# corelab-src/dacapo

Hardware: AMD Instinct MI355X
Metric: NTT/s (NTT-equivalents over one run() of the ResNet HEVM program, nt=2^14) (higher is better)
Workload: dtype u64; 1 GPU; ResNet-20 (SiLU) HEVM program traced from the reference's examples/benchmarks/ResNet.py with its resnet20.silu.model weights, nt=2^14 slots, N=2^15, 14 x 60-bit primes (SEAL_HEVM.cpp:39-53); one independent ciphertext stream per GPU; streams_per_gpu=1, parallelism=replicas x1 (no collective in the op path)

## Files before the change

dacapo_amd/csrc/fused_ks.hip:

```cpp
#include "ks_mac.hpp"

namespace dacapo {

struct SrcStrided {
    const u64 *base;
    long stride;
    int prime_base, period;
    __device__ int prime(int z) const { return prime_base + z % period; }
    __device__ u64 load(int z, int g, int) const { return base[(long)z * stride + g]; }
};
template <int E>
__device__ __forceinline__ void rs_operand(u64 (&v)[E], const int (&g)[E], const RsItem &it, const SumSrc *__restrict__ srcs, int p, int i,
                                           size_t N, const DModulus &M)
{
    if (it.count == 0) {
        const u64 *x = it.src.limb(p, i, N);
#pragma unroll
        for (int j = 0; j < E; j++) v[j] = x[g[j]];
    } else {
        u64 s[E];
        Acc128 a[E];
#pragma unroll
        for (int j = 0; j < E; j++) s[j] = 0, a[j].clear();
        int n_plain = 0, n_prod = 0;
// ... 624 lines not shown
    const int z = blockIdx.y, k = z % t, b = z / t;
    const size_t N = (size_t)1 << logN;
    const double ratio = items[b].ratio;
    const u64 *cf = pt + (size_t)b * ELL * N;
    u64 *out = ptx + (size_t)z * N;
    const DModulus M = mods[k];
    ntt_tile<K, LOGE, true, false, false>(
        M, tw + ((size_t)k << logN), logN, blockIdx.x,
        [=](int g) { return residue_of_double(reencoded_coeff_fixed<ELL>(cf, (size_t)g, N, mods, crt, ratio), M); },
        [=](int g, u64 v) { out[g] = v; }, lds);
}

template <int K, int LOGE>
__global__ __launch_bounds__(kTileThreads) void f_frows_boot_final_kernel(const u64 *__restrict__ ptx, const BootItem *__restrict__ items,
                                                                           int t, const DModulus *__restrict__ mods,
                                                                           const u64 *__restrict__ tw, int logN)
{
    __shared__ __attribute__((aligned(16))) u64 lds[TileGeo<LOGE>::LDS_ELEMS];
    const int z = blockIdx.y, i = z % t;
    const size_t N = (size_t)1 << logN;
    const BootItem it = items[z / t];
    const DModulus M = mods[i];
    const u64 *in = ptx + (size_t)z * N;
    const u64 *z0 = it.zenc + (size_t)i * N, *z1 = it.zenc + ((size_t)t + i) * N;
    u64 *o0 = it.dst.limb(0, i, N), *o1 = it.dst.limb(1, i, N);
    ntt_tile<K, LOGE, false, false, true>(
        M, tw + ((size_t)i << logN), logN, blockIdx.x, [=](int g) { return in[g]; },
        [=](int g, u64 v) {
            o0[g] = addmod(v, z0[g], M.q);
            o1[g] = z1[g];
        },
        lds);
}

template <class Src>
static void launch_irows(const Context &c, Src src, u64 *out, long out_stride, int count, hipStream_t s)
{
    DC_GEO_SWITCH(c.k2, count, DC_LAUNCH((f_irows_kernel<KK, LE, Src>), grid, dim3(kTileThreads), 0, s, src, out, out_stride,
                                                  c.d_mods, c.d_itw, c.logN));
// ... 49 lines not shown
{
    DC_GEO_SWITCH(c.k2, B * ell, DC_LAUNCH((f_irows_boot_kernel<KK, LE>), grid, dim3(kTileThreads), 0, s, items, srcs, sk, ell, out,
                                                    c.d_mods, c.d_itw, c.logN));
}
void f_boot_reencode_fcols(const Context &c, const u64 *pt, u64 *ptx, const BootItem *items, int B, int ell, int t, CrtDev crt,
                           hipStream_t s)
{
    if (ell == 1) {
        DC_GEO_SWITCH(c.k1, B * t, DC_LAUNCH((f_boot_reencode_fcols_kernel<KK, LE, 1>), grid, dim3(kTileThreads), 0, s, pt, ptx, items,
                                                      t, c.d_mods, crt, c.d_tw, c.logN));
    } else {
        fprintf(stderr, "[dacapo_amd] f_boot_reencode_fcols: source level %d not instantiated\n", ell);
        abort();
    }
}
void f_frows_boot_final(const Context &c, const u64 *ptx, const BootItem *items, int B, int t, hipStream_t s)
{
    DC_GEO_SWITCH(c.k2, B * t, DC_LAUNCH((f_frows_boot_final_kernel<KK, LE>), grid, dim3(kTileThreads), 0, s, ptx, items, t,
                                                  c.d_mods, c.d_tw, c.logN));
}

void f_ks_frows_mac(const Context &c, int mode, const u64 *ext, const u64 *target, const KsItem *items, const u64 *shared_key, u64 *acc,
                    int B, int ell, hipStream_t s, bool fold_base)
{
    const u64 *pmod = (fold_base && mode == 0) ? c.d_pmod : nullptr;
    const KsMacShape sh = ks_mac_shape(c, ell, B);
    ks_mac_dispatch(c.k2, sh, [&](auto k, auto le, auto merge) {
        constexpr int KK = decltype(k)::value, LE = decltype(le)::value;
        constexpr bool MG = decltype(merge)::value;
        if (mode == 0)
            DC_LAUNCH((f_ks_frows_mac_kernel<KK, LE, 0, MG>), sh.grid, dim3(kTileThreads), 0, s, ext, target, items, shared_key, acc, ell, c.K,
                      c.d_mods, c.d_tw, c.d_itw, c.logN, pmod, sh.items_fast);
        else
            DC_LAUNCH((f_ks_frows_mac_kernel<KK, LE, 1, MG>), sh.grid, dim3(kTileThreads), 0, s, ext, target, items, shared_key, acc, ell, c.K,
// ... 102 lines not shown
```

dacapo_amd/csrc/hevm_vm.hip:

```cpp
#include "hevm_vm.hpp"

#include "../../include/dacapo_ckks.h"
#include "c_api_types.hpp"
#include "chacha.hpp"
#include "seal_serial.hpp"

#include <math.h>
#include <string.h>
#include <sys/random.h>

#include <algorithm>
#include <cmath>
#include <chrono>
#include <fstream>
#include <iostream>

namespace dacapo {

constexpr int kVmThreads = 256;

constexpr int kRngCoefs = 8;

__device__ __forceinline__ int rng_cbd(u64 w)
{
// ... 39 lines not shown

__global__ __launch_bounds__(kVmThreads) void sample_small_kernel(u64 *__restrict__ out, size_t N, int limbs, int cbd, ChaChaKey key,
                                                                   u64 object, u32 domain, const DModulus *__restrict__ mods)
{
    const size_t blk = (size_t)blockIdx.x * kVmThreads + threadIdx.x;
    u64 w[kRngCoefs];
    rng_words8(key, object, blk, 0, 0, domain, w);
    int v[kRngCoefs];
#pragma unroll
    for (int e = 0; e < kRngCoefs; e++) v[e] = cbd ? rng_cbd(w[e]) : rng_ternary(w[e]);
    for (int i = 0; i < limbs; i++) store_small8(out + (size_t)i * N + blk * kRngCoefs, v, mods[i].q);
}

__global__ __launch_bounds__(kVmThreads) void sample_enc_batch_kernel(u64 *__restrict__ out, size_t N, int cnt, ChaChaKey key, u64 object0,
                                                                       const DModulus *__restrict__ mods,
                                                                       const u64 *__restrict__ epoch)
{
    const int b = blockIdx.y / 3, z = blockIdx.y % 3;
    const size_t blk = (size_t)blockIdx.x * kVmThreads + threadIdx.x;
    u64 w[kRngCoefs];
    rng_words8(key, object0 + (u64)b, blk, *epoch, 0, RNG_ENC_U + (u32)z, w);
    int v[kRngCoefs];
#pragma unroll
    for (int e = 0; e < kRngCoefs; e++) v[e] = z ? rng_cbd(w[e]) : rng_ternary(w[e]);
    for (int i = 0; i < cnt; i++) store_small8(out + (((size_t)b * 3 + z) * cnt + i) * N + blk * kRngCoefs, v, mods[i].q);
}

__global__ void chacha_blocks_kernel(u32 *__restrict__ out, ChaChaKey key, u64 counter, u64 nonce, int blocks)
{
    const int b = blockIdx.x * blockDim.x + threadIdx.x;
    if (b >= blocks) return;
    u32 o[16];
    chacha20_block(key, counter + (u64)b, nonce, o);
    for (int i = 0; i < 16; i++) out[b * 16 + i] = o[i];
}

// ... 317 lines not shown
    encoder.reset(new HostEncoder(logN));
    use_plan = option(OPT_PLAN) != 0;
    plan_graph = option(OPT_PLAN_GRAPH) != 0;
    plan_dag = option(OPT_PLAN_GRAPH) == 2;
    plan_lanes = option(OPT_PLAN_LANES) >= 2 ? 2 : 1;
    host_encoder = option(OPT_HOST_ENCODER) != 0;
    fold_rescale_into_boot = option(OPT_FOLD_RESCALE_BOOT) != 0;
    lazy_sums = option(OPT_HYB_LAZY_SUM) != 0;
    double_hoist = (lazy_sums && option(OPT_HYB_DOUBLE_HOIST) != 0) || ks_lazy == 2;
    max_batch = std::max(1, (int)option(OPT_MAX_BATCH));
    chain_fusion = option(OPT_CHAIN_FUSION) != 0;
    secret_weight = (int)option(OPT_SECRET_HW);
    boot_secret_weight = (int)option(OPT_BOOT_SECRET_HW);
    rot_compose = option(OPT_ROT_COMPOSE) != 0;
    online_encode = option(OPT_ONLINE_ENCODE) != 0 && use_plan && !host_encoder;
    lanes.resize(1);
    DC_HIP_CHECK(hipStreamCreateWithFlags(&lanes[0].stream, hipStreamNonBlocking));
    lanes[0].ws = ctx->ws0;
    lanes[0].boot_plain.d = dalloc((size_t)ctx->max_level() * ctx->N);
    lanes[0].boot_plain.level = ctx->max_level();
    DC_HIP_CHECK(vm_malloc(&d_epoch, 8));
    DC_HIP_CHECK(hipMemset(d_epoch, 0, 8));
    cur = 0;
}

void HEVM::gen_kswitch_key(u64 *key, const u64 *new_key, u64 key_id) { gen_kswitch_key_in(*ctx, key, keys.sk, new_key, key_id); }

void HEVM::gen_kswitch_key_in(Context &c, u64 *key, const u64 *key_sk, const u64 *new_key, u64 key_id)
{
    const size_t N = c.N;
    const int K = c.K;
    const dim3 gu((unsigned)(N / (kRngCoefs * kVmThreads)), (unsigned)K), gs((unsigned)(N / (kRngCoefs * kVmThreads))),
        g2((unsigned)(N / (2 * kVmThreads)), (unsigned)K);
    const int L = c.max_level();
    for (int j = 0; j < c.key_digits(); j++) {
        u64 *c0 = key + (size_t)j * 2 * K * N, *c1 = c0 + (size_t)K * N;
        const u64 object = key_id * 64 + (u64)j;
// ... 735 lines not shown
    const size_t N = c.N;
    const int ell = pt.level, cnt = ell + 1;
    if (!keys.pk) {
        fprintf(stderr, "[dacapo_amd] encrypt: this VM has no public key\n");
        abort();
    }
    if (test_zero_enc) {
        DC_HIP_CHECK(hipMemcpyAsync(dst.data, pt.d, (size_t)ell * N * 8, hipMemcpyDeviceToDevice, S()));
        DC_HIP_CHECK(hipMemsetAsync(dst.data + dst.poly_stride, 0, (size_t)ell * N * 8, S()));
        dst.level = ell, dst.scale = pt.scale;
        return;
    }
    u64 *ue = W().ks_ext;
    const CtView tmp{ dst.data, (long)dst.poly_stride };
    DC_LAUNCH(sample_enc_batch_kernel, dim3((unsigned)(N / (kRngCoefs * kVmThreads)), 3), dim3(kVmThreads), 0, S(), ue, N, cnt,
                       rng.secret, enc_counter++, c.d_mods, d_epoch);
    launch_ntt(c, false, ue, (long)N, 3 * cnt, nullptr, 0, cnt, S());
    DC_LAUNCH(pk_encrypt_kernel, dim3((unsigned)(N / (2 * kVmThreads)), (unsigned)cnt, 2), dim3(kVmThreads), 0, S(),
                       tmp.p, tmp.poly_stride, keys.pk, (long)c.K * (long)N, ue, ue + (size_t)cnt * N, (long)cnt * (long)N, N, c.d_mods);
    rescale_fused(c, W(), tmp, tmp, cnt, pt.d, S());
    dst.level = ell;
    dst.scale = pt.scale;
}

void HEVM::encrypt(int64_t i, const double *dat, int len)
{
    Plain pt;
    encode_internal(pt, dat, (size_t)len, (int)arg_level.at((size_t)i), (int)arg_scale.at((size_t)i));
    hevm_ctxt &r = reg((size_t)i);
    reg_base[(size_t)i] = home[(size_t)i];
    r.data = reg_base[(size_t)i] + (size_t)sel * (size_t)2 * ctx->K * ctx->N;
// ... 450 lines not shown
    const CrtTables &tb = crt_tables(ell);
    u64 *pt = W().ks_tmp;
    u64 *lohi = W().ks_digits;
    f_irows_decrypt(c, src, keys.sk, ell, pt, S());
    launch_ntt_cols_inv(c, pt, (long)N, ell, nullptr, 0, 0, S());
    const CrtDev cd{ tb.inv, tb.mmod, tb.hmod, tb.hdig, tb.mdbl };
    DC_LAUNCH(reencode_kernel, dim3((unsigned)((N / 2 + kVmThreads) / kVmThreads)), dim3(kVmThreads), 0, S(), lohi,
                       lohi + N, pt, ell, N, c.d_mods, cd, new_scale / src_scale);
    Plain ptx{ lanes[cur].boot_plain.d, target_level, new_scale };
    DC_LAUNCH(lift_i128_kernel, dim3((unsigned)(N / kVmThreads), (unsigned)target_level), dim3(kVmThreads), 0, S(),
                       ptx.d, lohi, lohi + N, N, c.d_mods);
    launch_ntt(c, false, ptx.d, (long)N, target_level, nullptr, 0, 0, S());
    encrypt_plain(dst, ptx);
}

void HEVM::plan_zero_encrypt(int first, int B, int t, hipStream_t s)
{
    Context &c = *ctx;
    const size_t N = c.N;
    const int cnt = t + 1;
    if (!keys.pk) {
        fprintf(stderr, "[dacapo_amd] bootstrap: this VM has no public key\n");
        abort();
    }
    Plan &P = plan;
    DC_LAUNCH(sample_enc_batch_kernel, dim3((unsigned)(N / (kRngCoefs * kVmThreads)), (unsigned)(3 * B)), dim3(kVmThreads), 0, s,
                       P.boot_ue, N, cnt, rng.secret, ((u64)1 << 32) + (u64)first, c.d_mods, d_epoch);
    launch_ntt(c, false, P.boot_ue, (long)N, 3 * cnt * B, nullptr, 0, cnt, s);
    DC_LAUNCH(pk_encrypt_batch_kernel, dim3((unsigned)(N / (2 * kVmThreads)), (unsigned)cnt, (unsigned)(2 * B)), dim3(kVmThreads),
                       0, s, P.boot_tmp, keys.pk, (long)c.K * (long)N, P.boot_ue, cnt, N, c.d_mods);
    b_rescale(c, P.ws[0], P.d_boot_rs + first, B, cnt, s);
}

void HEVM::plan_boot_step(int first, int B, int ell, int t, int lane, hipStream_t s, const Handoff &h)
{
    Context &c = *ctx;
    const size_t N = c.N;
    if (!keys.sk) {
        fprintf(stderr, "[dacapo_amd] bootstrap: needs a full VM (secret + public key)\n");
        abort();
    }
    Plan &P = plan;
    const BootItem *items = P.d_boot + first;
    const CrtTables &tb = crt_tables(ell);
    const CrtDev cd{ tb.inv, tb.mmod, tb.hmod, tb.hdig, tb.mdbl };
    u64 *pt = P.boot_pt[lane], *ptx = P.boot_ptx[lane];
    if (h.in)
        pt = const_cast<u64 *>(h.in);
    else
        f_irows_decrypt_items(c, items, P.d_sum_srcs, keys.sk, ell, pt, B, s);
    launch_ntt_cols_inv(c, pt, (long)N, B * ell, nullptr, 0, ell, s);
    if (ell == 1)
        f_boot_reencode_fcols(c, pt, ptx, items, B, ell, t, cd, s);
    else {
        DC_LAUNCH(reencode_lift_batch_kernel, dim3((unsigned)((N / 2 + kVmThreads) / kVmThreads), (unsigned)B), dim3(kVmThreads), 0,
                           s, ptx, pt, items, ell, t, N, c.d_mods, cd);
        launch_ntt_cols_fwd(c, ptx, (long)N, B * t, nullptr, 0, t, s);
    }
    f_frows_boot_final(c, ptx, items, B, t, s);
}

void HEVM::dispatch(const WireOp &op)
{
    switch (op.opcode) {
    case 1: op_rotate(op.dst, op.lhs, (int16_t)op.rhs); break;
    case 2: op_negate(op.dst, op.lhs); break;
    case 3: op_rescale(op.dst, op.lhs); break;
    case 4: op_modswitch(op.dst, op.lhs, (int16_t)op.rhs); break;
    case 5: fprintf(stderr, "This VM does not support native upscale op\n"); abort();
    case 6: op_addcc(op.dst, op.lhs, op.rhs); break;
    case 7: op_addcp(op.dst, op.lhs, op.rhs); break;
    case 8: op_mulcc(op.dst, op.lhs, op.rhs); break;
    case 9: op_mulcp(op.dst, op.lhs, op.rhs); break;
    case 10: op_bootstrap(op.dst, op.lhs, op.rhs); break;
// ... 12 lines not shown
    n_hops = n_decomp = 0;
    t_bootstrap = 0.0;
    int i = (int)((header.hevm_header_size + config.config_body_length) / 8), j = 0;
    for (const WireOp &op : ops) {
        if (debug) {
            std::cout << std::endl;
            std::cout << std::oct << i++ << " " << std::dec << j++ << std::endl;
            std::cout << "opcode [" << op.opcode << "], dst [" << op.dst << "], lhs [" << op.lhs << "], rhs [" << op.rhs << "]"
                      << std::endl;
        }
        if (op.opcode <= 10) op_counts[op.opcode]++;
        if (op.opcode == 0 || (op.opcode > 10 && (op.opcode < kOpConj || op.opcode > kOpKeySwitch))) continue;
        dispatch(op);
    }
    bump_epoch(S());
}

void HEVM::run()
{
    if (use_plan && !debug) {
        run_plan();
        return;
    }
    if (streams != 1) {
        fprintf(stderr, "[dacapo_amd] several ciphertext streams need the batched plan (option plan = 1, no debug)\n");
        abort();
    }
    execute();
    DC_HIP_CHECK(hipStreamSynchronize(S()));
}

}

namespace dacapo {
thread_local VmAllocs *g_vm_allocs = nullptr;

void HEVM::destroy_device_state()
{
    (void)hipDeviceSynchronize();
    drop_plan_graph();
    for (Lane &ln : lanes)
        if (ln.stream) (void)hipStreamDestroy(ln.stream), ln.stream = nullptr;
    if (aux_stream) (void)hipStreamDestroy(aux_stream), aux_stream = nullptr;
    for (hipEvent_t e : plan.events) (void)hipEventDestroy(e);
    plan.events.clear();
    const std::vector<void *> live(allocs.live.begin(), allocs.live.end());
    allocs.live.clear();
    for (void *p : live) (void)hipFree(p);
}
}

using dacapo::HEVM;
static HEVM *V(void *vm)
{
    HEVM *h = static_cast<HEVM *>(vm);
// ... 348 lines not shown
```

dacapo_amd/csrc/hevm_vm.hpp:

```cpp
#pragma once
#include "wire_parse.hpp"
#include <complex>
#include <deque>
#include <map>
#include <set>
#include <memory>
#include <string>
#include <unordered_set>
#include <vector>

#include "../../include/hevm_abi.h"
#include "chacha.hpp"
#include "seal_serial.hpp"
#include "kernels.hpp"
#include "encoder.hpp"
#include "plan.hpp"

namespace dacapo {

struct VmAllocs {
    std::unordered_set<void *> live;
};
extern thread_local VmAllocs *g_vm_allocs;
template <class T>
// ... 158 lines not shown
        SumGroupSrc *d_sumg_srcs = nullptr;
        CtView *d_cont_other = nullptr;
        struct EncGroup { int wave, level, first, count; u64 *out; };
        std::vector<EncGroup> enc_groups;
        EncItem *d_enc_items = nullptr;
        u64 *enc_arena = nullptr;
        double2 *enc_scratch = nullptr;
        int *d_enc_overflow = nullptr;
        size_t enc_arena_bytes = 0, enc_scratch_bytes = 0;
        std::vector<EwItem> h_ew;
        std::vector<u64 *> handoff_bufs;
        size_t n_fused = 0;
        BootItem *d_boot = nullptr;
        RsItem *d_boot_rs = nullptr;
        size_t zenc_bytes = 0;
        u64 *zenc = nullptr, *boot_ue = nullptr, *boot_tmp = nullptr, *boot_pt[2] = { nullptr, nullptr }, *boot_ptx[2] = { nullptr, nullptr };
        struct BootChunk { int first, count, target; };
        std::vector<BootChunk> boot_chunks;
        BatchWs ws[2];
        std::vector<hipEvent_t> events;
        std::vector<u64 *> pool;
        int64_t n_keyswitch = 0, n_ntt = 0;
        int64_t n_hops = 0, n_decomp = 0;
        size_t launches = 0, max_live = 0;
        hipGraph_t graph = nullptr;
        hipGraphExec_t graph_exec = nullptr;
    } plan;
    bool plan_graph = true;
    bool plan_dag = false;
    void capture_plan();
// ... 1 lines not shown
    void issue_step(const Step &st, hipStream_t q);
    void drop_plan_graph();
    void issue_plan(hipStream_t s);
    bool use_plan = true;
    bool test_zero_enc = false;
    int max_batch = 64;
    std::vector<u64 *> home;
    int streams = 1, sel = 0;
    std::vector<u64 *> reg_base;
    void set_streams(int n);
    void select_stream(int s);
    void build_plan();
    void run_plan();
    void boot_item(CtView src, int src_level, double src_scale, hevm_ctxt &dst, int target_level);
    void plan_zero_encrypt(int first, int B, int t, hipStream_t s);
    void plan_boot_step(int first, int B, int ell, int t, int lane, hipStream_t s, const Handoff &h);
    bool rot_compose = false;
    std::vector<int> compose_rotation(int steps) const;
    mutable std::vector<int> rot_offsets;
    mutable std::set<int> rot_offset_set;
    mutable size_t rot_offsets_epoch = (size_t)-1;
    int boot_secret_weight = 0;
    int secret_weight = 0;
    bool ks_hoist = false;
    int ks_lazy = 0;
    KsItem *d_hoist_items = nullptr;
    void rotate_hop_vm(CtView dst, CtView src, u32 elt, const u64 *key, int ell);
    bool chain_fusion = true;
    hipStream_t aux_stream = nullptr;
    bool double_hoist = false;
// ... 63 lines not shown
```

dacapo_amd/csrc/options.cpp:

```cpp
#include "options.hpp"

#include "../../include/hevm_abi.h"

#include <stdio.h>
#include <stdlib.h>
#include <string.h>

namespace dacapo {

struct OptDef {
    const char *name;
    long long def;
};
static const OptDef kDefs[OPT_COUNT] = {
    { "logn", 15 },
    { "primes", 14 },
    { "prime_bits", 60 },
    { "ks_special", 1 },
    { "ks_alpha", 0 },
    { "secret_hw", 0 },
    { "boot_secret_hw", 0 },
    { "rot_compose", 0 },
    { "plan", 1 },
    { "plan_graph", 1 },
    { "plan_lanes", 2 },
    { "plan_aux_min_cost", 3 },
    { "max_batch", 64 },
    { "chain_fusion", 1 },
    { "host_encoder", 0 },
    { "online_encode", 0 },
    { "fold_rescale_boot", 0 },
    { "hyb_mfma", 1 },
    { "hyb_fuse", 2 },
    { "hyb_lazy_sum", 0 },
    { "hyb_double_hoist", 0 },
    { "ks_hoist", 0 },
    { "ks_lazy_sum", 0 },
    { "seal_compr", 0 },
    { "trace", 0 },
    { "step_profile", 0 },
    { "small_tile_wgs", -1 },
    { "tiny_tile_wgs", 2000 },
    { "wide_tile_wgs", 2048 },
    { "rows_prime_major", 16 },
    { "ntt_full_min_limbs", 768 },
    { "ntt_full_inv_min_limbs", 768 },
    { "ntt_full_persist", -1 },
    { "ntt_full_inv_persist", -1 },
    { "ntt_full_pairs", 1 },
    { "ntt_full_inv_pairs", 1 },
    { "cols_pairs", 1 },
    { "ks_merge_special_min_wgs", 2048 },
// ... 118 lines not shown
```

dacapo_amd/csrc/options.hpp:

```cpp
#pragma once

namespace dacapo {

enum Opt : int {
    OPT_LOGN,
    OPT_PRIMES,
    OPT_PRIME_BITS,
    OPT_KS_SPECIAL,
    OPT_KS_ALPHA,
    OPT_SECRET_HW,
    OPT_BOOT_SECRET_HW,
    OPT_ROT_COMPOSE,
    OPT_PLAN,
    OPT_PLAN_GRAPH,
    OPT_PLAN_LANES,
    OPT_PLAN_AUX_MIN_COST,
    OPT_MAX_BATCH,
    OPT_CHAIN_FUSION,
    OPT_HOST_ENCODER,
    OPT_ONLINE_ENCODE,
    OPT_FOLD_RESCALE_BOOT,
    OPT_HYB_MFMA,
    OPT_HYB_FUSE,
    OPT_HYB_LAZY_SUM,
    OPT_HYB_DOUBLE_HOIST,
    OPT_KS_HOIST,
    OPT_KS_LAZY_SUM,
    OPT_SEAL_COMPR,
    OPT_TRACE,
    OPT_STEP_PROFILE,
    OPT_SMALL_TILE_WGS,
    OPT_TINY_TILE_WGS,
    OPT_WIDE_TILE_WGS,
    OPT_ROWS_PRIME_MAJOR,
    OPT_NTT_FULL_MIN_LIMBS,
    OPT_NTT_FULL_INV_MIN_LIMBS,
    OPT_NTT_FULL_PERSIST,
    OPT_NTT_FULL_INV_PERSIST,
    OPT_NTT_FULL_PAIRS,
    OPT_NTT_FULL_INV_PAIRS,
    OPT_COLS_PAIRS,
    OPT_KS_MERGE_SPECIAL_MIN_WGS,
// ... 14 lines not shown
```

dacapo_amd/csrc/plan.hpp:

```cpp
#pragma once
#include "crt_device.hpp"
#include "kernels.hpp"

namespace dacapo {

struct KsItem {
    CtView src, dst;
    const u64 *key;
    u32 elt;
    u32 slot;
    const u64 *plain = nullptr, *plain_sp = nullptr;
};
struct MulItem {
    CtView a, b, dst;
};
struct RsItem {
    CtView src, dst;
    int first = 0, count = 0;
    const u64 *add = nullptr;
    const u64 *mul = nullptr;
};
struct EwItem {
    CtView dst, a, b;
};
// ... 73 lines not shown
void b_sum(Context &c, const SumItem *d_items, const SumSrc *d_srcs, int B, int ell, hipStream_t s);
void b_sum_group(Context &c, const SumGroup *d_groups, const SumGroupSrc *d_gsrcs, int G, int ell, hipStream_t s);
void modraise(Context &c, u64 *scratch, const EwItem *h_items, int B, int target, hipStream_t s, const EwItem *d_items = nullptr);

void f_irows_strided(const Context &c, const u64 *base, long stride, int prime_base, int period, u64 *out, long out_stride, int count,
                     hipStream_t s);
void f_irows_rot_c1(const Context &c, const KsItem *items, int ell, u64 *out, int B, hipStream_t s);
void f_irows_rs_last(const Context &c, const RsItem *items, const SumSrc *srcs, int l, u64 *out, int B, hipStream_t s);
void f_irows_rs_single(const Context &c, CtView src, int l, u64 *out, hipStream_t s);
void f_irows_decrypt(const Context &c, CtView ct, const u64 *sk, int ell, u64 *out, hipStream_t s);
void f_irows_tensor_c2(const Context &c, const MulItem *items, int ell, u64 *out, int B, hipStream_t s);
void f_irows_decrypt_items(const Context &c, const BootItem *items, const SumSrc *srcs, const u64 *sk, int ell, u64 *out, int B,
                           hipStream_t s);
void f_boot_reencode_fcols(const Context &c, const u64 *pt, u64 *ptx, const BootItem *items, int B, int ell, int t, CrtDev crt,
                           hipStream_t s);
void f_frows_boot_final(const Context &c, const u64 *ptx, const BootItem *items, int B, int t, hipStream_t s);
void f_ks_icols_lift_fcols(const Context &c, const u64 *digits, u64 *ext, int B, int ell, hipStream_t s);
void f_dr_icols_lift_fcols(const Context &c, const u64 *last, long last_stride, u64 *tmp, int polys, int cnt, int l, hipStream_t s);
void f_ks_frows_mac(const Context &c, int mode, const u64 *ext, const u64 *target, const KsItem *items, const u64 *shared_key, u64 *acc,
                    int B, int ell, hipStream_t s, bool fold_base = false);
void f_ks_lift_fcols(const Context &c, const u64 *digits, u64 *ext, int B, int ell, hipStream_t s);
void f_dr_lift_fcols(const Context &c, const u64 *last, long last_stride, u64 *tmp, int polys, int cnt, int l, hipStream_t s);
void f_frows_final(const Context &c, int mode, const u64 *tmp, const void *items, const u64 *acc, int polys, int cnt, int l,
                   hipStream_t s, RsItem single = RsItem{}, const u64 *plain = nullptr, const SumSrc *srcs = nullptr,
                   const Handoff &h = Handoff{}, bool base_folded = false);
void rescale_fused(Context &c, const Workspace &w, CtView dst, CtView src, int ell, const u64 *plain, hipStream_t s);

}
```

dacapo_amd/csrc/plan_exec.hip:

```cpp
#include <math.h>
#include <string.h>

#include <algorithm>
#include <chrono>
#include <map>
#include <functional>
#include <queue>
#include <set>
#include <tuple>

#include "hevm_vm.hpp"

namespace dacapo {

#define ks_ntts(ell) ks_ntt_count(c, (ell))

template <class T>
static T *upload(const std::vector<T> &v)
{
    T *d = nullptr;
    DC_HIP_CHECK(vm_malloc(&d, std::max<size_t>(v.size(), 1) * sizeof(T)));
    if (!v.empty()) DC_HIP_CHECK(hipMemcpy(d, v.data(), v.size() * sizeof(T), hipMemcpyHostToDevice));
    return d;
}

void HEVM::build_plan()
{
    Context &c = *ctx;
    const size_t N = c.N;
    Plan &P = plan;
    for (u64 *b : P.handoff_bufs) (void)vm_free(b);
    P.handoff_bufs.clear();
    for (void *p : { (void *)P.d_enc_items, (void *)P.enc_arena, (void *)P.enc_scratch, (void *)P.d_enc_overflow })
        if (p) (void)vm_free(p);
    P.d_enc_items = nullptr, P.enc_arena = nullptr, P.enc_scratch = nullptr, P.d_enc_overflow = nullptr;
    P.enc_groups.clear(), P.enc_arena_bytes = P.enc_scratch_bytes = 0;
    if (P.d_cont_other) (void)vm_free(P.d_cont_other), P.d_cont_other = nullptr;
    for (void *p : { (void *)P.d_ks, (void *)P.d_mul, (void *)P.d_rs, (void *)P.d_ew, (void *)P.d_sum, (void *)P.d_sum_srcs, (void *)P.d_sumg, (void *)P.d_sumg_srcs, (void *)P.d_boot,
                     (void *)P.d_boot_rs, (void *)P.zenc, (void *)P.boot_ue, (void *)P.boot_tmp, (void *)P.boot_pt[0], (void *)P.boot_ptx[0],
                     (void *)P.boot_pt[1], (void *)P.boot_ptx[1] })
        if (p) (void)vm_free(p);
    P.d_boot = nullptr, P.d_boot_rs = nullptr, P.zenc = P.boot_ue = P.boot_tmp = nullptr;
    P.boot_pt[0] = P.boot_pt[1] = P.boot_ptx[0] = P.boot_ptx[1] = nullptr;
    P.boot_chunks.clear();
    if (P.graph_exec) (void)hipGraphExecDestroy(P.graph_exec);
    if (P.graph) (void)hipGraphDestroy(P.graph);
    P.graph_exec = nullptr, P.graph = nullptr;
    P.vals.clear(), P.pops.clear(), P.steps.clear();
    P.n_keyswitch = P.n_ntt = 0;
    P.n_hops = P.n_decomp = 0;
    const size_t nreg = ciphers.size();
    const int S = streams;
    std::vector<int> cur(nreg, -1);
    auto new_val = [&](int level, double scale) {
        Val v;
        v.level = level, v.scale = scale, v.root = (int)P.vals.size();
        P.vals.push_back(v);
// ... 863 lines not shown
        for (int pi : step_pops[s]) {
            const Pop &p = O[(size_t)pi];
            for (int v : p.srcs) st.reads.push_back(V[(size_t)V[(size_t)v].root].buf);
            st.writes.push_back(V[(size_t)V[(size_t)p.dst].root].buf);
        }
        if (st.fused_consumer >= 0 && st.h.cont == CONT_MUL)
            for (int pi : step_pops[(size_t)st.fused_consumer])
                for (int v : O[(size_t)pi].srcs) st.reads.push_back(V[(size_t)V[(size_t)v].root].buf);
        for (auto *vec : { &st.reads, &st.writes }) {
            std::sort(vec->begin(), vec->end());
            vec->erase(std::unique(vec->begin(), vec->end()), vec->end());
        }
    }
    if (!h_boot_pops.empty()) {
        const size_t nb = h_boot_pops.size(), slot = (size_t)2 * boot_tmax * N;
        DC_HIP_CHECK(vm_malloc(&P.zenc, nb * slot * sizeof(u64)));
        P.zenc_bytes = nb * slot * sizeof(u64);
        std::vector<int> order(nb);
        for (size_t i = 0; i < nb; i++) order[i] = (int)i;
        std::stable_sort(order.begin(), order.end(), [&](int a, int b) {
            return O[(size_t)h_boot_pops[(size_t)a].first].target_level < O[(size_t)h_boot_pops[(size_t)b].first].target_level;
        });
        const size_t bc = std::min<size_t>(nb, (size_t)std::max(max_batch, 1));
        const size_t cmax = (size_t)boot_tmax + 1;
        DC_HIP_CHECK(vm_malloc(&P.boot_ue, bc * 3 * cmax * N * sizeof(u64)));
        DC_HIP_CHECK(vm_malloc(&P.boot_tmp, bc * 2 * cmax * N * sizeof(u64)));
        for (int ln = 0; ln < plan_lanes; ln++) {
            DC_HIP_CHECK(vm_malloc(&P.boot_pt[ln], std::max<size_t>(need_bpt, 1) * N * sizeof(u64)));
            DC_HIP_CHECK(vm_malloc(&P.boot_ptx[ln], std::max<size_t>(need_bptx, 1) * N * sizeof(u64)));
        }
        std::vector<BootItem> h_boot(nb);
        std::vector<RsItem> h_brs(nb);
        for (size_t k = 0; k < nb;) {
            const int t = O[(size_t)h_boot_pops[(size_t)order[k]].first].target_level;
            size_t e = k;
            while (e < nb && e - k < bc && O[(size_t)h_boot_pops[(size_t)order[e]].first].target_level == t) e++;
            P.boot_chunks.push_back({ (int)k, (int)(e - k), t });
            for (size_t j = k; j < e; j++) {
                const size_t item = (size_t)order[j];
                u64 *z = P.zenc + item * slot;
                h_brs[j] = RsItem{ CtView{ P.boot_tmp + (j - k) * 2 * (size_t)(t + 1) * N, (long)(t + 1) * (long)N }, CtView{ z, (long)t * (long)N } };
// ... 13 lines not shown
            } else
                src_scale = V[(size_t)p.srcs[0]].scale;
            bi.ratio = new_scale / src_scale;
            if (p.rs_sum) {
                bi.first = (int)h_srcs.size(), bi.count = (int)p.srcs.size();
                for (size_t k = 0; k < p.srcs.size(); k++) {
                    const int pl = p.src_plain.empty() ? -1 : p.src_plain[k];
                    h_srcs.push_back(SumSrc{ view(p.srcs[k], q), pl >= 0 ? plains.at((size_t)pl).d : nullptr });
                }
            }
            if (p.rs_add >= 0) bi.add = plains.at((size_t)p.rs_add).d;
            if (p.rs_mul >= 0) bi.mul = plains.at((size_t)p.rs_mul).d;
            h_boot[item] = bi;
        }
        P.d_boot = upload(h_boot), P.d_boot_rs = upload(h_brs);
    }
    P.d_ks = upload(h_ks), P.d_mul = upload(h_mul), P.d_rs = upload(h_rs), P.d_ew = upload(h_ew), P.d_sum = upload(h_sum);
    P.h_ew = h_ew;
    P.d_sum_srcs = upload(h_srcs);
    P.d_sumg = upload(h_sumg), P.d_sumg_srcs = upload(h_sumg_srcs);
    {
        std::vector<size_t> other_first(P.steps.size(), 0);
        for (size_t ai = 0; ai < P.steps.size(); ai++) {
            Step &A = P.steps[ai];
            if (A.fused_consumer < 0) continue;
            Step &B = P.steps[(size_t)A.fused_consumer];
            const size_t items = (size_t)B.count, limbs = A.h.cont == CONT_RS ? 2 : (size_t)B.level;
            u64 *buf = nullptr;
            DC_HIP_CHECK(vm_malloc(&buf, items * limbs * N * sizeof(u64)));
            P.handoff_bufs.push_back(buf);
// ... 128 lines not shown
            b_sum(c, P.d_sum + st.first, P.d_sum_srcs, st.count, st.level, q);
        break;
    case P_NEG: b_ew(c, EwOp::Neg, P.d_ew + st.first, st.count, 2, 2, st.level, q); break;
    case P_COPY: b_ew(c, EwOp::Copy, P.d_ew + st.first, st.count, 2, 2, st.level, q); break;
    case P_MODRAISE: modraise(c, w.digits, P.h_ew.data() + st.first, st.count, st.target, q, P.d_ew + st.first); break;
    case P_MULP: b_ew(c, EwOp::Mul, P.d_ew + st.first, st.count, 2, 1, st.level, q); break;
    case P_ADDP: b_add_plain(c, P.d_ew + st.first, st.count, st.level, q); break;
    case P_BOOT: plan_boot_step(st.first, st.count, st.level, st.target, st.lane, q, st.h); break;
    }
}

void HEVM::issue_plan(hipStream_t s)
{
    Context &c = *ctx;
    Plan &P = plan;
    if (test_zero_enc) {
        if (P.zenc) DC_HIP_CHECK(hipMemsetAsync(P.zenc, 0, P.zenc_bytes, s));
    } else
        for (const Plan::BootChunk &bc : P.boot_chunks) plan_zero_encrypt(bc.first, bc.count, bc.target, s);
    const bool step_profile = option(OPT_STEP_PROFILE) != 0 && !plan_graph;
    std::map<std::tuple<int, int, int>, std::pair<int, double>> prof;
    double wave_max = 0, wave_sum = 0, crit_path = 0, all_steps = 0;
    size_t waves_seen = 0, wide_waves = 0;
    size_t ev = 0, eg = 0;
    for (size_t a = 0; a < P.steps.size();) {
        size_t b = a;
        bool has_aux = false;
        while (b < P.steps.size() && P.steps[b].wave == P.steps[a].wave) has_aux |= P.steps[b].lane == 1, b++;
        for (; eg < P.enc_groups.size() && P.enc_groups[eg].wave <= P.steps[a].wave; eg++) {
            const Plan::EncGroup &g = P.enc_groups[eg];
            enc_batch(c, enc_tables, online.d_consts, P.d_enc_items + g.first, g.count, g.level, P.enc_scratch, g.out, P.d_enc_overflow, s);
// ... 108 lines not shown
                DC_HIP_CHECK(hipGraphKernelNodeGetParams(cur, &kp));
                DC_HIP_CHECK(hipGraphAddKernelNode(&nw, main, dp, nd, &kp));
            } else if (ty == hipGraphNodeTypeMemset) {
                hipMemsetParams mp;
                DC_HIP_CHECK(hipGraphMemsetNodeGetParams(cur, &mp));
                DC_HIP_CHECK(hipGraphAddMemsetNode(&nw, main, dp, nd, &mp));
            } else
                ok = false;
            tail = nw;
            auto it = next.find(cur);
            cur = it == next.end() ? nullptr : it->second;
        }
        (void)hipGraphDestroy(g);
        return tail;
    };
    hipGraphNode_t zenc_tail = add_unit([&](hipStream_t s) {
        if (test_zero_enc) {
            if (P.zenc) DC_HIP_CHECK(hipMemsetAsync(P.zenc, 0, P.zenc_bytes, s));
        } else
            for (const Plan::BootChunk &bc : P.boot_chunks) plan_zero_encrypt(bc.first, bc.count, bc.target, s);
    }, {});
    struct Ref { int lane = -1; long seq = -1; hipGraphNode_t node = nullptr; };
    std::map<const u64 *, Ref> writer;
    std::map<const u64 *, Ref> reader[2];
    Ref lane_tail[2] = { Ref{ 0, 0, zenc_tail }, Ref{ 1, 0, zenc_tail } };
    long seq = 0;
    for (size_t i = 0; i < P.steps.size() && ok; i++) {
        const Step &st = P.steps[i];
        const int other = 1 - st.lane;
        Ref cross;
        auto need = [&](const Ref &r) {
// ... 38 lines not shown

void HEVM::run_plan()
{
    if (!plan.ready) build_plan();
    Context &c = *ctx;
    Plan &P = plan;
    cur = 0;
    hipStream_t s = S();
    memset(op_counts, 0, sizeof(op_counts));
    for (const WireOp &op : ops)
        if (op.opcode <= 10) op_counts[op.opcode]++;
    n_keyswitch = P.n_keyswitch, n_ntt = P.n_ntt;
    n_hops = P.n_hops, n_decomp = P.n_decomp;
    t_bootstrap = 0.0;
    const long ps = (long)c.K * (long)c.N;
    if (plan_graph) {
        capture_plan();
        if (P.graph_exec)
            DC_HIP_CHECK(hipGraphLaunch(P.graph_exec, s));
        else
            issue_plan(s);
    } else
        issue_plan(s);
    DC_HIP_CHECK(hipStreamSynchronize(s));
    if (P.d_enc_overflow) {
        int overflow = 0;
        DC_HIP_CHECK(hipMemcpy(&overflow, P.d_enc_overflow, sizeof(int), hipMemcpyDeviceToHost));
        if (overflow) {
            fprintf(stderr, "[dacapo_amd] encode: coefficient does not fit 120 bits (scale too large)\n");
            abort();
        }
    }
    for (size_t r = 0; r < P.final_val.size() && r < ciphers.size(); r++) {
        const int v = P.final_val[r];
        if (v < 0) continue;
        reg_base[r] = P.vals[(size_t)P.vals[(size_t)v].root].buf;
        ciphers[r].data = reg_base[r] + (size_t)sel * (size_t)2 * c.K * c.N;
        ciphers[r].poly_stride = ps;
        ciphers[r].level = P.vals[(size_t)v].level;
// ... 6 lines not shown
```

Baseline: 1.290 million NTT/s.

## Prefetch next run's bootstrap zero-encryptions on a low-priority side stream

Double-buffers the zero-encryption arena used by bootstrapping and indexes it by epoch parity. While the current run's plan graph executes, the next epoch's zero-encryptions are produced in chunks on a separate low-priority stream, so they no longer sit serially at the start of the plan. This adds memory for a second arena and side-stream scratch buffers. It also creates contention between the side-stream kernels and the main plan, plus a host sync on the side stream at the end of each run.

```diff
diff --git a/dacapo_amd/csrc/fused_ks.hip b/dacapo_amd/csrc/fused_ks.hip
--- a/dacapo_amd/csrc/fused_ks.hip
+++ b/dacapo_amd/csrc/fused_ks.hip
@@ -662,7 +662,8 @@
 template <int K, int LOGE>
 __global__ __launch_bounds__(kTileThreads) void f_frows_boot_final_kernel(const u64 *__restrict__ ptx, const BootItem *__restrict__ items,
                                                                            int t, const DModulus *__restrict__ mods,
-                                                                           const u64 *__restrict__ tw, int logN)
+                                                                           const u64 *__restrict__ tw, int logN,
+                                                                           const u64 *__restrict__ epoch, size_t arena_stride)
 {
     __shared__ __attribute__((aligned(16))) u64 lds[TileGeo<LOGE>::LDS_ELEMS];
     const int z = blockIdx.y, i = z % t;
@@ -670,7 +671,8 @@
     const BootItem it = items[z / t];
     const DModulus M = mods[i];
     const u64 *in = ptx + (size_t)z * N;
-    const u64 *z0 = it.zenc + (size_t)i * N, *z1 = it.zenc + ((size_t)t + i) * N;
+    const u64 *zenc = it.zenc + (epoch ? (size_t)(*epoch & 1) * arena_stride : 0);
+    const u64 *z0 = zenc + (size_t)i * N, *z1 = zenc + ((size_t)t + i) * N;
     u64 *o0 = it.dst.limb(0, i, N), *o1 = it.dst.limb(1, i, N);
     ntt_tile<K, LOGE, false, false, true>(
         M, tw + ((size_t)i << logN), logN, blockIdx.x, [=](int g) { return in[g]; },
@@ -750,10 +752,10 @@
         abort();
     }
 }
-void f_frows_boot_final(const Context &c, const u64 *ptx, const BootItem *items, int B, int t, hipStream_t s)
+void f_frows_boot_final(const Context &c, const u64 *ptx, const BootItem *items, int B, int t, hipStream_t s, const u64 *epoch, size_t arena_stride)
 {
     DC_GEO_SWITCH(c.k2, B * t, DC_LAUNCH((f_frows_boot_final_kernel<KK, LE>), grid, dim3(kTileThreads), 0, s, ptx, items, t,
-                                                  c.d_mods, c.d_tw, c.logN));
+                                                  c.d_mods, c.d_tw, c.logN, epoch, arena_stride));
 }
 
 void f_ks_frows_mac(const Context &c, int mode, const u64 *ext, const u64 *target, const KsItem *items, const u64 *shared_key, u64 *acc,
diff --git a/dacapo_amd/csrc/hevm_vm.hip b/dacapo_amd/csrc/hevm_vm.hip
--- a/dacapo_amd/csrc/hevm_vm.hip
+++ b/dacapo_amd/csrc/hevm_vm.hip
@@ -77,12 +77,12 @@
 
 __global__ __launch_bounds__(kVmThreads) void sample_enc_batch_kernel(u64 *__restrict__ out, size_t N, int cnt, ChaChaKey key, u64 object0,
                                                                        const DModulus *__restrict__ mods,
-                                                                       const u64 *__restrict__ epoch)
+                                                                       const u64 *__restrict__ epoch, u64 epoch_val)
 {
     const int b = blockIdx.y / 3, z = blockIdx.y % 3;
     const size_t blk = (size_t)blockIdx.x * kVmThreads + threadIdx.x;
     u64 w[kRngCoefs];
-    rng_words8(key, object0 + (u64)b, blk, *epoch, 0, RNG_ENC_U + (u32)z, w);
+    rng_words8(key, object0 + (u64)b, blk, epoch ? *epoch : epoch_val, 0, RNG_ENC_U + (u32)z, w);
     int v[kRngCoefs];
 #pragma unroll
     for (int e = 0; e < kRngCoefs; e++) v[e] = z ? rng_cbd(w[e]) : rng_ternary(w[e]);
@@ -430,6 +430,8 @@
     boot_secret_weight = (int)option(OPT_BOOT_SECRET_HW);
     rot_compose = option(OPT_ROT_COMPOSE) != 0;
     online_encode = option(OPT_ONLINE_ENCODE) != 0 && use_plan && !host_encoder;
+    zenc_prefetch = option(OPT_ZENC_PREFETCH) != 0 && use_plan;
+    zenc_chunk = std::max(1, (int)option(OPT_ZENC_PREFETCH_CHUNK));
     lanes.resize(1);
     DC_HIP_CHECK(hipStreamCreateWithFlags(&lanes[0].stream, hipStreamNonBlocking));
     lanes[0].ws = ctx->ws0;
@@ -437,6 +439,7 @@
     lanes[0].boot_plain.level = ctx->max_level();
     DC_HIP_CHECK(vm_malloc(&d_epoch, 8));
     DC_HIP_CHECK(hipMemset(d_epoch, 0, 8));
+    h_epoch = 0;
     cur = 0;
 }
 
@@ -1202,7 +1205,7 @@
     u64 *ue = W().ks_ext;
     const CtView tmp{ dst.data, (long)dst.poly_stride };
     DC_LAUNCH(sample_enc_batch_kernel, dim3((unsigned)(N / (kRngCoefs * kVmThreads)), 3), dim3(kVmThreads), 0, S(), ue, N, cnt,
-                       rng.secret, enc_counter++, c.d_mods, d_epoch);
+                       rng.secret, enc_counter++, c.d_mods, d_epoch, (u64)0);
     launch_ntt(c, false, ue, (long)N, 3 * cnt, nullptr, 0, cnt, S());
     DC_LAUNCH(pk_encrypt_kernel, dim3((unsigned)(N / (2 * kVmThreads)), (unsigned)cnt, 2), dim3(kVmThreads), 0, S(),
                        tmp.p, tmp.poly_stride, keys.pk, (long)c.K * (long)N, ue, ue + (size_t)cnt * N, (long)cnt * (long)N, N, c.d_mods);
@@ -1683,7 +1686,9 @@
     encrypt_plain(dst, ptx);
 }
 
-void HEVM::plan_zero_encrypt(int first, int B, int t, hipStream_t s)
+void HEVM::plan_zero_encrypt(int first, int B, int t, hipStream_t s) { zero_encrypt_range(first, B, t, 0, s, false, d_epoch, 0); }
+
+void HEVM::zero_encrypt_range(int first, int B, int t, int off, hipStream_t s, bool side, const u64 *epoch_ptr, u64 epoch)
 {
     Context &c = *ctx;
     const size_t N = c.N;
@@ -1693,12 +1698,24 @@
         abort();
     }
     Plan &P = plan;
+    u64 *ue = side ? P.zside_ue : P.boot_ue;
+    u64 *tmp = (side ? P.zside_tmp : P.boot_tmp) + (size_t)off * 2 * (size_t)cnt * N;
+    const RsItem *rs = epoch_ptr ? P.d_boot_rs : P.d_zrs[side ? 1 : 0][epoch & 1];
     DC_LAUNCH(sample_enc_batch_kernel, dim3((unsigned)(N / (kRngCoefs * kVmThreads)), (unsigned)(3 * B)), dim3(kVmThreads), 0, s,
-                       P.boot_ue, N, cnt, rng.secret, ((u64)1 << 32) + (u64)first, c.d_mods, d_epoch);
-    launch_ntt(c, false, P.boot_ue, (long)N, 3 * cnt * B, nullptr, 0, cnt, s);
+                       ue, N, cnt, rng.secret, ((u64)1 << 32) + (u64)(first + off), c.d_mods, epoch_ptr, epoch);
+    launch_ntt(c, false, ue, (long)N, 3 * cnt * B, nullptr, 0, cnt, s);
     DC_LAUNCH(pk_encrypt_batch_kernel, dim3((unsigned)(N / (2 * kVmThreads)), (unsigned)cnt, (unsigned)(2 * B)), dim3(kVmThreads),
-                       0, s, P.boot_tmp, keys.pk, (long)c.K * (long)N, P.boot_ue, cnt, N, c.d_mods);
-    b_rescale(c, P.ws[0], P.d_boot_rs + first, B, cnt, s);
+                       0, s, tmp, keys.pk, (long)c.K * (long)N, ue, cnt, N, c.d_mods);
+    b_rescale(c, side ? P.zside_ws : P.ws[0], rs + first + off, B, cnt, s);
+}
+
+void HEVM::zero_encrypt_set(hipStream_t s, bool side, u64 epoch)
+{
+    for (const Plan::BootChunk &bc : plan.boot_chunks) {
+        const int piece = side ? std::max(1, std::min(zenc_chunk, bc.count)) : bc.count;
+        for (int off = 0; off < bc.count; off += piece)
+            zero_encrypt_range(bc.first, std::min(piece, bc.count - off), bc.target, off, s, side, nullptr, epoch);
+    }
 }
 
 void HEVM::plan_boot_step(int first, int B, int ell, int t, int lane, hipStream_t s, const Handoff &h)
@@ -1726,7 +1743,7 @@
                            s, ptx, pt, items, ell, t, N, c.d_mods, cd);
         launch_ntt_cols_fwd(c, ptx, (long)N, B * t, nullptr, 0, t, s);
     }
-    f_frows_boot_final(c, ptx, items, B, t, s);
+    f_frows_boot_final(c, ptx, items, B, t, s, P.zenc_stride ? d_epoch : nullptr, P.zenc_stride);
 }
 
 void HEVM::dispatch(const WireOp &op)
@@ -1769,6 +1786,7 @@
         dispatch(op);
     }
     bump_epoch(S());
+    h_epoch++;
 }
 
 void HEVM::run()
@@ -1792,8 +1810,10 @@
 
 void HEVM::destroy_device_state()
 {
+    if (zenc_stream) (void)hipStreamSynchronize(zenc_stream);
     (void)hipDeviceSynchronize();
     drop_plan_graph();
+    if (zenc_stream) (void)hipStreamDestroy(zenc_stream), zenc_stream = nullptr;
     for (Lane &ln : lanes)
         if (ln.stream) (void)hipStreamDestroy(ln.stream), ln.stream = nullptr;
     if (aux_stream) (void)hipStreamDestroy(aux_stream), aux_stream = nullptr;
diff --git a/dacapo_amd/csrc/hevm_vm.hpp b/dacapo_amd/csrc/hevm_vm.hpp
--- a/dacapo_amd/csrc/hevm_vm.hpp
+++ b/dacapo_amd/csrc/hevm_vm.hpp
@@ -196,6 +196,12 @@
         BootItem *d_boot = nullptr;
         RsItem *d_boot_rs = nullptr;
         size_t zenc_bytes = 0;
+        size_t zenc_stride = 0;
+        RsItem *d_zrs[2][2] = { { nullptr, nullptr }, { nullptr, nullptr } };
+        u64 *zside_ue = nullptr, *zside_tmp = nullptr;
+        BatchWs zside_ws;
+        long long zenc_filled = -1;
+        bool zenc_zeroed = false;
         u64 *zenc = nullptr, *boot_ue = nullptr, *boot_tmp = nullptr, *boot_pt[2] = { nullptr, nullptr }, *boot_ptx[2] = { nullptr, nullptr };
         struct BootChunk { int first, count, target; };
         std::vector<BootChunk> boot_chunks;
@@ -227,6 +233,12 @@
     void run_plan();
     void boot_item(CtView src, int src_level, double src_scale, hevm_ctxt &dst, int target_level);
     void plan_zero_encrypt(int first, int B, int t, hipStream_t s);
+    bool zenc_prefetch = false;
+    int zenc_chunk = 32;
+    hipStream_t zenc_stream = nullptr;
+    u64 h_epoch = 0;
+    void zero_encrypt_set(hipStream_t s, bool side, u64 epoch);
+    void zero_encrypt_range(int first, int B, int t, int off, hipStream_t s, bool side, const u64 *epoch_ptr, u64 epoch);
     void plan_boot_step(int first, int B, int ell, int t, int lane, hipStream_t s, const Handoff &h);
     bool rot_compose = false;
     std::vector<int> compose_rotation(int steps) const;
diff --git a/dacapo_amd/csrc/options.cpp b/dacapo_amd/csrc/options.cpp
--- a/dacapo_amd/csrc/options.cpp
+++ b/dacapo_amd/csrc/options.cpp
@@ -36,6 +36,8 @@
     { "hyb_double_hoist", 0 },
     { "ks_hoist", 0 },
     { "ks_lazy_sum", 0 },
+    { "zenc_prefetch", 1 },
+    { "zenc_prefetch_chunk", 32 },
     { "seal_compr", 0 },
     { "trace", 0 },
     { "step_profile", 0 },
diff --git a/dacapo_amd/csrc/options.hpp b/dacapo_amd/csrc/options.hpp
--- a/dacapo_amd/csrc/options.hpp
+++ b/dacapo_amd/csrc/options.hpp
@@ -26,6 +26,8 @@
     OPT_HYB_DOUBLE_HOIST,
     OPT_KS_HOIST,
     OPT_KS_LAZY_SUM,
+    OPT_ZENC_PREFETCH,
+    OPT_ZENC_PREFETCH_CHUNK,
     OPT_SEAL_COMPR,
     OPT_TRACE,
     OPT_STEP_PROFILE,
diff --git a/dacapo_amd/csrc/plan.hpp b/dacapo_amd/csrc/plan.hpp
--- a/dacapo_amd/csrc/plan.hpp
+++ b/dacapo_amd/csrc/plan.hpp
@@ -111,7 +111,8 @@
                            hipStream_t s);
 void f_boot_reencode_fcols(const Context &c, const u64 *pt, u64 *ptx, const BootItem *items, int B, int ell, int t, CrtDev crt,
                            hipStream_t s);
-void f_frows_boot_final(const Context &c, const u64 *ptx, const BootItem *items, int B, int t, hipStream_t s);
+void f_frows_boot_final(const Context &c, const u64 *ptx, const BootItem *items, int B, int t, hipStream_t s, const u64 *epoch = nullptr,
+                        size_t arena_stride = 0);
 void f_ks_icols_lift_fcols(const Context &c, const u64 *digits, u64 *ext, int B, int ell, hipStream_t s);
 void f_dr_icols_lift_fcols(const Context &c, const u64 *last, long last_stride, u64 *tmp, int polys, int cnt, int l, hipStream_t s);
 void f_ks_frows_mac(const Context &c, int mode, const u64 *ext, const u64 *target, const KsItem *items, const u64 *shared_key, u64 *acc,
diff --git a/dacapo_amd/csrc/plan_exec.hip b/dacapo_amd/csrc/plan_exec.hip
--- a/dacapo_amd/csrc/plan_exec.hip
+++ b/dacapo_amd/csrc/plan_exec.hip
@@ -38,9 +38,13 @@
     if (P.d_cont_other) (void)vm_free(P.d_cont_other), P.d_cont_other = nullptr;
     for (void *p : { (void *)P.d_ks, (void *)P.d_mul, (void *)P.d_rs, (void *)P.d_ew, (void *)P.d_sum, (void *)P.d_sum_srcs, (void *)P.d_sumg, (void *)P.d_sumg_srcs, (void *)P.d_boot,
                      (void *)P.d_boot_rs, (void *)P.zenc, (void *)P.boot_ue, (void *)P.boot_tmp, (void *)P.boot_pt[0], (void *)P.boot_ptx[0],
-                     (void *)P.boot_pt[1], (void *)P.boot_ptx[1] })
+                     (void *)P.boot_pt[1], (void *)P.boot_ptx[1], (void *)P.d_zrs[0][0], (void *)P.d_zrs[0][1], (void *)P.d_zrs[1][0], (void *)P.d_zrs[1][1],
+                     (void *)P.zside_ue, (void *)P.zside_tmp, (void *)P.zside_ws.digits, (void *)P.zside_ws.tmp })
         if (p) (void)vm_free(p);
     P.d_boot = nullptr, P.d_boot_rs = nullptr, P.zenc = P.boot_ue = P.boot_tmp = nullptr;
+    P.d_zrs[0][0] = P.d_zrs[0][1] = P.d_zrs[1][0] = P.d_zrs[1][1] = nullptr;
+    P.zside_ue = P.zside_tmp = nullptr, P.zside_ws = BatchWs{};
+    P.zenc_stride = 0, P.zenc_filled = -1, P.zenc_zeroed = false;
     P.boot_pt[0] = P.boot_pt[1] = P.boot_ptx[0] = P.boot_ptx[1] = nullptr;
     P.boot_chunks.clear();
     if (P.graph_exec) (void)hipGraphExecDestroy(P.graph_exec);
@@ -934,8 +938,10 @@
     }
     if (!h_boot_pops.empty()) {
         const size_t nb = h_boot_pops.size(), slot = (size_t)2 * boot_tmax * N;
-        DC_HIP_CHECK(vm_malloc(&P.zenc, nb * slot * sizeof(u64)));
+        const bool two = zenc_prefetch;
+        DC_HIP_CHECK(vm_malloc(&P.zenc, (two ? 2 : 1) * nb * slot * sizeof(u64)));
         P.zenc_bytes = nb * slot * sizeof(u64);
+        P.zenc_stride = two ? nb * slot : 0;
         std::vector<int> order(nb);
         for (size_t i = 0; i < nb; i++) order[i] = (int)i;
         std::stable_sort(order.begin(), order.end(), [&](int a, int b) {
@@ -945,6 +951,17 @@
         const size_t cmax = (size_t)boot_tmax + 1;
         DC_HIP_CHECK(vm_malloc(&P.boot_ue, bc * 3 * cmax * N * sizeof(u64)));
         DC_HIP_CHECK(vm_malloc(&P.boot_tmp, bc * 2 * cmax * N * sizeof(u64)));
+        if (two) {
+            DC_HIP_CHECK(vm_malloc(&P.zside_ue, bc * 3 * cmax * N * sizeof(u64)));
+            DC_HIP_CHECK(vm_malloc(&P.zside_tmp, bc * 2 * cmax * N * sizeof(u64)));
+            DC_HIP_CHECK(vm_malloc(&P.zside_ws.digits, bc * 2 * N * sizeof(u64)));
+            DC_HIP_CHECK(vm_malloc(&P.zside_ws.tmp, bc * 2 * cmax * N * sizeof(u64)));
+            if (!zenc_stream) {
+                int lo = 0, hi = 0;
+                DC_HIP_CHECK(hipDeviceGetStreamPriorityRange(&lo, &hi));
+                DC_HIP_CHECK(hipStreamCreateWithPriority(&zenc_stream, hipStreamNonBlocking, lo));
+            }
+        }
         for (int ln = 0; ln < plan_lanes; ln++) {
             DC_HIP_CHECK(vm_malloc(&P.boot_pt[ln], std::max<size_t>(need_bpt, 1) * N * sizeof(u64)));
             DC_HIP_CHECK(vm_malloc(&P.boot_ptx[ln], std::max<size_t>(need_bptx, 1) * N * sizeof(u64)));
@@ -988,6 +1005,16 @@
             h_boot[item] = bi;
         }
         P.d_boot = upload(h_boot), P.d_boot_rs = upload(h_brs);
+        if (two)
+            for (int sc = 0; sc < 2; sc++)
+                for (int ar = 0; ar < 2; ar++) {
+                    std::vector<RsItem> v = h_brs;
+                    for (RsItem &it : v) {
+                        if (sc) it.src.p = P.zside_tmp + (it.src.p - P.boot_tmp);
+                        it.dst.p += (size_t)ar * P.zenc_stride;
+                    }
+                    P.d_zrs[sc][ar] = upload(v);
+                }
     }
     P.d_ks = upload(h_ks), P.d_mul = upload(h_mul), P.d_rs = upload(h_rs), P.d_ew = upload(h_ew), P.d_sum = upload(h_sum);
     P.h_ew = h_ew;
@@ -1146,7 +1173,8 @@
 {
     Context &c = *ctx;
     Plan &P = plan;
-    if (test_zero_enc) {
+    if (zenc_prefetch) {
+    } else if (test_zero_enc) {
         if (P.zenc) DC_HIP_CHECK(hipMemsetAsync(P.zenc, 0, P.zenc_bytes, s));
     } else
         for (const Plan::BootChunk &bc : P.boot_chunks) plan_zero_encrypt(bc.first, bc.count, bc.target, s);
@@ -1285,7 +1313,7 @@
         (void)hipGraphDestroy(g);
         return tail;
     };
-    hipGraphNode_t zenc_tail = add_unit([&](hipStream_t s) {
+    hipGraphNode_t zenc_tail = zenc_prefetch ? nullptr : add_unit([&](hipStream_t s) {
         if (test_zero_enc) {
             if (P.zenc) DC_HIP_CHECK(hipMemsetAsync(P.zenc, 0, P.zenc_bytes, s));
         } else
@@ -1354,15 +1382,31 @@
     n_hops = P.n_hops, n_decomp = P.n_decomp;
     t_bootstrap = 0.0;
     const long ps = (long)c.K * (long)c.N;
-    if (plan_graph) {
-        capture_plan();
-        if (P.graph_exec)
-            DC_HIP_CHECK(hipGraphLaunch(P.graph_exec, s));
-        else
-            issue_plan(s);
-    } else
+    if (plan_graph) capture_plan();
+    const bool prefetch = zenc_prefetch && !P.boot_chunks.empty();
+    bool fill = false;
+    if (prefetch) {
+        if (test_zero_enc) {
+            if (!P.zenc_zeroed) DC_HIP_CHECK(hipMemsetAsync(P.zenc, 0, 2 * P.zenc_bytes, s));
+            P.zenc_zeroed = true, P.zenc_filled = -1;
+        } else {
+            if (P.zenc_filled != (long long)h_epoch) zero_encrypt_set(s, false, h_epoch);
+            fill = true;
+        }
+    }
+    if (plan_graph && P.graph_exec) {
+        DC_HIP_CHECK(hipGraphLaunch(P.graph_exec, s));
+        if (fill) zero_encrypt_set(zenc_stream, true, h_epoch + 1);
+    } else {
+        if (fill) zero_encrypt_set(zenc_stream, true, h_epoch + 1);
         issue_plan(s);
+    }
     DC_HIP_CHECK(hipStreamSynchronize(s));
+    if (fill) {
+        DC_HIP_CHECK(hipStreamSynchronize(zenc_stream));
+        P.zenc_filled = (long long)(h_epoch + 1);
+    }
+    h_epoch++;
     if (P.d_enc_overflow) {
         int overflow = 0;
         DC_HIP_CHECK(hipMemcpy(&overflow, P.d_enc_overflow, sizeof(int), hipMemcpyDeviceToHost));
```

Result: no change. 1.305 million NTT/s, median of 4 (+1.2%).
